# eloj/radix-sorting

Measured on AMD Instinct MI355X. Metric: Gkeys/s sorting 2^28 u32 (1 GPU) + HBM GB/s vs roofline; 1/2/4/8-GPU scaling, higher is better.
Workload: dtype u32

## Files before the change

radix_sorting_amd/csrc/rsx.hip:

```cpp
#include "../../include/rsx.h"
#include "rsx_kernels.hpp"
#include "rsx_scatter2.hpp"
#include "rsx_small.hpp"
#include "rsx_hybrid.hpp"
#include "rsx_leaf16.hpp"
#include "rsx_pass16.hpp"
#include "rsx_pass32.hpp"
#include "rsx_leafc.hpp"
#include "rsx_logroute.hpp"
#include "rsx_pass64.hpp"
#include "rsx_unique.hpp"
#include "rsx_group.hpp"
#include "rsx_topk.hpp"
#include "rsx_nth.hpp"
#include "rsx_lex.hpp"

#include <hip/hip_runtime.h>

#include <algorithm>
#include <cstdarg>
#include <cstdio>
#include <cstdlib>
#include <cstring>
#include <map>
// ... 653 lines not shown
}

template <typename KT> constexpr u64 seg_extra_rows() { return sizeof(KT) == 8 ? 512 : 256; }

template <typename KT> bool pass64a_narrow_wanted(const Ctx &c)
{
	if (sizeof(KT) != 8 || !narrow_slots_ok<KT>(c.slack_cap) || env().no_pass64a || env().no_unstable || !c.slack_mean)
		return false;
	u32 r = 0;
	while ((u64)(r + 1) * (r + 1) <= c.slack_mean)
		++r;
	return c.slack_mean + 6 * (r + 1) + 8 <= c.slack_cap - Pass2wCfg<u32>::BACK;
}

template <typename KT>
int launch_seg_pass(Ctx &c, const KT *aux, KT *src, size_t n, KdfArgs<KT> ka, int j, int blind = 0)
{
	typedef Sc2Cfg<KT, NoVal> C2;
	const u64 rows = (n + C2::TILE - 1) / C2::TILE + seg_extra_rows<KT>();
	const size_t st_bytes = 256 + rows * 256 * 4;
	char *base = (char *)c.seg.p + c.seg_status_off + (size_t)(blind == 1 ? 1 : j < 0 ? 0 : j) * st_bytes;
	SegArgs sa{};
	sa.ctl = (const SegCtl *)c.seg.p;
	sa.hist = (const u32 *)((char *)c.seg.p + c.seg_hist_off);
	sa.tiles = (const SegTile *)((char *)c.seg.p + c.seg_tiles_off);
	sa.slots = (u32)sizeof(KT) - 1;
	sa.slack_cap = blind == 1 ? c.slack1_cap : j == -2 ? c.slack_cap : 0u;
	sa.overflow = &((SegCtl *)c.seg.p)->overflow;
	KT *const second = blind == 1 ? src : blind == 2 ? const_cast<KT *>(aux) : nullptr;
	if (j == -2)
		src = (KT *)c.slack.p;
// ... 6 lines not shown
				const uintptr_t base_a = std::min(lo_a, hi_a);
				sa.out_off_lo = (u32)((lo_a - base_a) / sizeof(KT));
				sa.out_off_hi = (u32)((hi_a - base_a) / sizeof(KT));
				first = (KT *)base_a;
			} else {
				sa.kin_hi = (const void *)hi_a;
				first = second;
			}
		}
		if (blind == 1)
			src = first;
		else
			aux = first;
	}
	const bool dense = sizeof(KT) == 4 && blind == 2 && dense_slots<KT>(c);
	ProfScope prof(dense ? 3 : 1, (u64)n * (dense ? sizeof(KT) + 2 : 2 * sizeof(KT)), c.stream);
	const bool plain = ka.fmask == 0 && ka.sflip == 0 && ka.desc == 0;
	u32 flags = j == -2 ? (u32)SCATTER_SEG_SLACK : j < 0 ? (u32)SCATTER_SEG_LEAVES : 0u;
	if (blind)
		flags |= SCATTER_BLIND | (blind == 1 ? (u32)SCATTER_BLIND_TOP : 0u);
	if (blind && !env().no_unstable)
		flags |= SCATTER_UNSTABLE;
	const u32 pi = j < 0 ? 0u : (u32)j;
	const unsigned grid = blind == 1 ? (unsigned)(rows - seg_extra_rows<KT>()) : (unsigned)rows;
	const u32 shift0 = 0u;
#define RSX_LAUNCH_SEG(DIGV)                                                                                               \
	hipLaunchKernelGGL((rsx_scatter2_kernel<KT, NoVal, u32, C2, false, DIGV, false, KT, true>), dim3(grid),                 \
	                   dim3(C2::BLOCK), 0, c.stream, aux, src, (const NoVal *)nullptr, (NoVal *)nullptr, (u64)n, shift0,     \
	                   (const u64 *)c.ghist(), 1u, (u32 *)(base + 256), (u32 *)base, ka, flags, (u64 *)nullptr,             \
	                   (const Plan *)c.plan(), pi, 0u, (const u32 *)nullptr, sa)
	if constexpr (sizeof(KT) == 4) {
		if (dense && pass16a_wanted<KT>(c)) {
			const unsigned pgrid = 512;
			if (plain)
				hipLaunchKernelGGL((rsx_pass16a_kernel<KT, DIG_PLAIN>), dim3(pgrid), dim3(Pass16aCfg::BLOCK), 0, c.stream, (const KT *)aux,
				                   (const KT *)sa.kin_hi, sa.lo_slots, (unsigned short *)src, sa.tiles, sa.ctl, (const Plan *)c.plan(),
				                   (u32 *)(base + 256), sa.slack_cap, sa.overflow, ka);
			else
				hipLaunchKernelGGL((rsx_pass16a_kernel<KT, DIG_GENERIC>), dim3(pgrid), dim3(Pass16aCfg::BLOCK), 0, c.stream, (const KT *)aux,
				                   (const KT *)sa.kin_hi, sa.lo_slots, (unsigned short *)src, sa.tiles, sa.ctl, (const Plan *)c.plan(),
				                   (u32 *)(base + 256), sa.slack_cap, sa.overflow, ka);
			HIP_TRY(hipGetLastError());
			return RSX_OK;
		}
		if (dense && !env().no_pass16 && !env().no_unstable && !env().no_leaf16) {
			const u32 *btile = (const u32 *)((char *)c.seg.p + c.seg_btile_off);
#define RSX_LAUNCH_P16(DIGV, CFG)                                                                                          \
	hipLaunchKernelGGL((rsx_pass16_kernel<KT, DIGV, CFG>), dim3(grid), dim3(CFG::BLOCK), 0, c.stream, (const KT *)aux,      \
	                   (const KT *)sa.kin_hi, sa.lo_slots, (unsigned short *)src, sa.tiles, btile, sa.ctl,                  \
// ... 358 lines not shown
	u32 *btile = (u32 *)((char *)c.seg.p + c.seg_btile_off);
	u64 *off1 = (u64 *)c.gscan.p;
	if (!c.seg_ev && !c.small.external)
		HIP_TRY(hipEventCreateWithFlags(&c.seg_ev, hipEventDisableTiming));
	if (c.host_segctl)
		c.host_segctl->mode = SEG_MODE_NONE;
	c.slack1_cap = cap1;
	c.slack_cap = cap2;
	const bool atoms = pass16a_wanted<KT>(c);
	const bool atoms64 = pass64a_narrow_wanted<KT>(c);
	typedef Pass32aCfgT<sizeof(KT) == 8 ? 14 : 28> P32;
	const size_t min32 = env().pass32_min_mi ? (size_t)env().pass32_min_mi << 20 : sizeof(KT) == 8 ? (size_t)3 << 23 : (size_t)13 << 22;
	const bool atoms1 = (sizeof(KT) == 4 ? atoms : !env().no_unstable) && !env().no_pass32a && n >= min32 &&
	                    cap1 >= (u32)P32::TILE + 2 * PASS32_BACK;
	const bool rep4 = (c.hints & 1u) != 0 || (env().probe & 4u) != 0;
	c.narrow1 = sizeof(KT) == 8 && atoms1 && atoms64 && lo != 0 && !rep4 && !env().no_narrow1 && (((uintptr_t)aux) & 63) == 0 &&
	            (size_t)256 * cap1 * 4 <= n * sizeof(KT);
	static_assert(sizeof(SegCtl) <= 256, "the control block is not part of what is zeroed");
	RSX_TRY(blind_forget_device_backoff(c));
	hipLaunchKernelGGL((rsx_blind_precheck_kernel<KT>), dim3(1 + 512), dim3(1024), 0, c.stream, (const KT *)src, (u64)n, ka, ctl,
	                   c.plan(), c.dev_host_plan, (u32x4 *)((char *)c.seg.p + c.seg_status_off), (u64)(2 * st_bytes / 16),
	                   4u,
	                   (u32)(sizeof(KT) == 4 && dense_slots<KT>(c) && !env().no_leaf16 && !env().no_shift ? 1 : 0),
	                   (u32)(narrow_slots_ok<KT>(cap2) ? (c.narrow1 ? 2 : 1) : 0), 0u,
	                   (u32)(g_in_async ? 1 : 0), (u32)((env().probe & 4u) ? 1u : c.hints));
	{
		if (atoms1) {
			u32 off_lo = 0, off_hi = 0;
			KT *kbase = (KT *)c.slack1.p;
			if (lo) {
				const uintptr_t lo_a = (uintptr_t)aux, hi_a = (uintptr_t)c.slack1.p - (size_t)lo * cap1 * sizeof(KT);
				const uintptr_t base_a = std::min(lo_a, hi_a);
				off_lo = (u32)((lo_a - base_a) / sizeof(KT));
				off_hi = (u32)((hi_a - base_a) / sizeof(KT));
				kbase = (KT *)base_a;
			}
			u32 *cur1 = (u32 *)((char *)c.seg.p + c.seg_status_off + st_bytes + 256);
			u32 *ovf = &((SegCtl *)c.seg.p)->overflow;
			const bool plain = ka.fmask == 0 && ka.sflip == 0 && ka.desc == 0;
			ProfScope prof(1, (u64)n * 2 * sizeof(KT), c.stream);
			const bool prefetch = sizeof(KT) == 4 && env().pass32_prefetch > 0;
#define RSX_LAUNCH_P32R(DIGV, PF, REPV)                                                                                      \
			hipLaunchKernelGGL((rsx_pass32a_kernel<KT, DIGV, PF, P32, REPV>), dim3(256), dim3(P32::BLOCK), 0, c.stream,              \
			                   (const KT *)src, (u64)n, kbase, lo, off_lo, off_hi, cap1, (const SegCtl *)ctl, cur1, ovf, ka)
#define RSX_LAUNCH_P32(DIGV, PF)                                                                                             \
			do {                                                                                                                 \
				if (rep4 && !(PF))                                                                                               \
					RSX_LAUNCH_P32R(DIGV, false, 4);                                                                             \
				else                                                                                                             \
					RSX_LAUNCH_P32R(DIGV, PF, 1);                                                                                \
			} while (0)
			if constexpr (sizeof(KT) == 4) {
				if (plain && prefetch)
					RSX_LAUNCH_P32(DIG_PLAIN, true);
				else if (!plain && prefetch)
					RSX_LAUNCH_P32(DIG_GENERIC, true);
			}
			if (plain && !prefetch)
				RSX_LAUNCH_P32(DIG_PLAIN, false);
			else if (!prefetch)
				RSX_LAUNCH_P32(DIG_GENERIC, false);
#undef RSX_LAUNCH_P32
#undef RSX_LAUNCH_P32R
			if constexpr (sizeof(KT) == 8) {
				if (c.narrow1) {
					if (plain)
						hipLaunchKernelGGL((rsx_pass32a_kernel<KT, DIG_PLAIN, false, P32, 1, u32>), dim3(256), dim3(P32::BLOCK), 0, c.stream,
						                   (const KT *)src, (u64)n, (u32 *)aux, 256u, 0u, 0u, cap1, (const SegCtl *)ctl, cur1, ovf, ka);
					else
						hipLaunchKernelGGL((rsx_pass32a_kernel<KT, DIG_GENERIC, false, P32, 1, u32>), dim3(256), dim3(P32::BLOCK), 0, c.stream,
						                   (const KT *)src, (u64)n, (u32 *)aux, 256u, 0u, 0u, cap1, (const SegCtl *)ctl, cur1, ovf, ka);
				}
			}
			HIP_TRY(hipGetLastError());
		}
	}
	if (!atoms1)
		RSX_TRY(launch_seg_pass<KT>(c, src, lo ? aux : nullptr, n, ka, -2, 1));
	hipLaunchKernelGGL(rsx_seg_tiles_kernel, dim3(32), dim3(256), 0, c.stream, (const u64 *)c.ghist(), (u64)n, (const Plan *)c.plan(),
	                   atoms ? (u32)Pass16aCfg::TILE : (u32)C2::TILE, tiles, ctl, btile, off1, cap1,
	                   (const u32 *)((char *)c.seg.p + c.seg_status_off + st_bytes + 256), (u32)ntiles0, atoms1 ? PASS32_BACK : 0u,
	                   atoms64 ? (u32)Pass2wCfg<u32>::TILE : 0u, c.narrow1 ? (u32)Pass64aCfgLow::TILE : 0u);
	RSX_TRY(launch_seg_pass<KT>(c, lo ? aux : nullptr, nullptr, n, ka, -2, 2));
	hipLaunchKernelGGL((rsx_seg_slack_plan_kernel<u32>), dim3(256), dim3(256), 0, c.stream,
	                   (const u32 *)((char *)c.seg.p + c.seg_status_off + 256), (const u32 *)btile, (const u64 *)c.ghist(),
	                   (const Plan *)c.plan(), ctl, segtab, cap2, c.dev_host_segctl, (const u64 *)off1,
	                   (atoms ? 2u : atoms64 ? 3u : 1u) | ((env().probe & 1u) << 8));
	HIP_TRY(hipGetLastError());
	if (c.seg_ev)
		HIP_TRY(hipEventRecord(c.seg_ev, c.stream));
	u32 leaf_shape = LeafShapes<KT>::shape_for_slots(cap2);
	if (dense_slots<KT>(c))
		leaf_shape |= 0x100u;
	if (sizeof(KT) == 8 && cap2 <= 5120u)
		leaf_shape |= 0x200u;
	RSX_TRY(launch_leaves<KT>(c, src, aux, n, ka, HYB_TWO_LEVEL, leaf_shape, (const u64 *)off1));
	*enqueued = 1;
	return RSX_OK;
// ... 1961 lines not shown
```

radix_sorting_amd/csrc/rsx_env.hpp:

```cpp
#pragma once

#include <algorithm>
#include <atomic>
#include <climits>
#include <cstdint>
#include <cstdlib>
#include <mutex>

namespace {

std::atomic<uint32_t> g_env_epoch{0};
enum : unsigned { UNIQUE_MAX_BITS_COMPILED = 30, UNIQUE_MAX_BITS_DEFAULT = 24 };
enum : unsigned { GROUP_MAX_BITS_COMPILED = 30, GROUP_MAX_BITS_DEFAULT = 24 };
enum : unsigned { LEX_PACK_BYTES_DEFAULT = 4 };
struct Env {
	bool host_register = false;
	bool force_table_rank = false;
	bool verify = false;
	bool verify_whole = false;
	bool verify_inject = false;
	bool no_hot = false;
	bool elem_loads = false;
	bool no_small_tiles = false;
	bool no_hybrid = false;
	bool no_small_sort = false;
	bool no_fill_runs = false;
	bool no_speculation = false;
	bool compact_bits = false;
	bool no_narrow_keys = false;
// ... 8 lines not shown
	bool no_leaf16q = false;
	bool no_narrow_slots = false;
	bool no_aux_slots = false;
	bool no_narrow1 = false;
	bool no_dense_slots = false;
	bool force_dense_slots = false;
	bool no_unstable = false;
	bool no_shift = false;
	bool no_pass16 = false;
	unsigned pass16_wgs = 2;
	bool no_packed_keys = false;
	bool no_pass32a = false;
	unsigned pass32_min_mi = 0;
	int pass32_prefetch = -1;
	bool no_pass16a = false;
	unsigned pass16_dbg = 0;
	bool no_leafc = false;
	unsigned force_leafc = 0;
	bool no_leaf16 = false;
	unsigned leaf16_maxbin = 25;
	unsigned leaf_grid = 65536;
	unsigned two_level_min_log2 = 27;
	bool no_odd_stride = false;
	unsigned cap1_pad_kib = 0;
	unsigned probe = 0;
	bool no_pass64a = false;
	bool no_log = false;
	bool log_leaf_big = false;
	bool pairs_leaf_big = false;
	unsigned log_min_log2 = 0;
// ... 55 lines not shown
		no_narrow1 = is_one("RSX_NO_NARROW_LEVEL1");
		no_dense_slots = is_one("RSX_NO_DENSE_SLOTS");
		force_dense_slots = is_one("RSX_DENSE_SLOTS");
		no_leaf16 = is_one("RSX_NO_LEAF16");
		no_leafc = is_one("RSX_NO_LEAFC");
		no_leaf16w2k = is_one("RSX_NO_LEAF16W2K");
		number("RSX_PASS32_MIN_MI", &pass32_min_mi);
		if (is_set("RSX_PASS32_PREFETCH"))
			pass32_prefetch = is_one("RSX_PASS32_PREFETCH");
		number("RSX_FORCE_LEAFC", &force_leafc);
		no_pass16 = is_one("RSX_NO_PASS16");
		no_pass16a = is_one("RSX_NO_PASS16A");
		no_pass32a = is_one("RSX_NO_PASS32A");
		no_packed_keys = is_one("RSX_NO_PACKED_KEYS");
		one_else_two("RSX_PASS16_WGS", &pass16_wgs);
		number("RSX_PASS16_DBG", &pass16_dbg);
		no_shift = is_one("RSX_NO_SHIFT");
		no_unstable = is_one("RSX_NO_UNSTABLE");
		number("RSX_LEAF16_MAXBIN", &leaf16_maxbin, 0, 25);
		number("RSX_LEAF_GRID", &leaf_grid, 256, 65536);
		no_odd_stride = is_one("RSX_NO_ODD_STRIDE");
		number("RSX_CAP1_PAD_KIB", &cap1_pad_kib, 0, 65536);
		number("RSX_PROBE", &probe);
		no_pass64a = is_one("RSX_NO_PASS64A");
		no_log = is_one("RSX_NO_LOG");
		log_leaf_big = is_one("RSX_LOG_LEAF_BIG");
		pairs_leaf_big = is_one("RSX_PAIRS_LEAF_BIG");
		number("RSX_LOG_MIN_LOG2", &log_min_log2, 20, 29);
		topk_force = one_or_two("RSX_TOPK_FORCE");
		nth_force = one_or_two("RSX_NTH_FORCE");
// ... 16 lines not shown
```

radix_sorting_amd/csrc/rsx_pass16.hpp:

```cpp
#pragma once

#include "rsx_kernels.hpp"
#include "rsx_hybrid.hpp"

namespace rsx {

template <int WGS_ = 2> struct Pass16Cfg {
	static constexpr int WGS = WGS_;
	static constexpr int BLOCK = 1024, KPT = 32, TILE = BLOCK * KPT;
	static constexpr int NGROUP = TILE / 8;
};

template <int WGS> struct Pass16Smem {
	__attribute__((aligned(16))) unsigned short stage[32768 + (WGS == 1 ? 8192 : 0)];
	u32 cell[256];
	u32 delta[256];
	unsigned short rend[256];
	unsigned char group_digit[4096];
	u32 wsum[4];
};

template <typename KT, int DIG, typename C = Pass16Cfg<2>>
__global__ __launch_bounds__(C::BLOCK, C::WGS * 4) void rsx_pass16_kernel(const KT *__restrict__ kin, const KT *__restrict__ kin_hi,
                                                                         u32 lo_slots, unsigned short *__restrict__ kout,
// ... 164 lines not shown
	static constexpr u32 BACK = 128;
	static constexpr int STAGE = TILE + 256 * 14;
};

struct Pass16aSmem {
	__attribute__((aligned(16))) unsigned short stage[Pass16aCfg::STAGE];
	__attribute__((aligned(16))) unsigned short carry[256][32];
	u32 cell[2][256];
	u32 delta[256];
	u32 info[256];
	unsigned short rbeg[256], bbeg[256], bend[256];
	unsigned char group_digit[Pass16aCfg::STAGE / 8];
	u32 wsum[4];
};

template <typename KT, int DIG, bool PREFETCH = false>
__global__ __launch_bounds__(Pass16aCfg::BLOCK, 8) void rsx_pass16a_kernel(const KT *__restrict__ kin, const KT *__restrict__ kin_hi,
                                                                          u32 lo_slots, unsigned short *__restrict__ kout,
                                                                          const SegTile *__restrict__ tiles,
                                                                          const SegCtl *__restrict__ ctl,
                                                                          const Plan *__restrict__ plan, u32 *__restrict__ cursors,
                                                                          u32 slack_cap, u32 *__restrict__ overflow, KdfArgs<KT> ka)
{
	static_assert(sizeof(KT) == 4, "4-byte keys, two-byte values");
	typedef Pass16aCfg C;
	constexpr int BLOCK = C::BLOCK, KPT = C::KPT, TILE = C::TILE;
	if (ctl->blind != BLIND_GO || plan->hyb != HYB_TWO_LEVEL)
		return;
	const u32 ntiles = ctl->ntiles;
	const u32 per = (ntiles + gridDim.x - 1) / gridDim.x;
	const u32 t0 = blockIdx.x * per, t1 = t0 + per < ntiles ? t0 + per : ntiles;
	if (t0 >= t1)
		return;
	const u32 shift = ctl->shift2;
	const u32 gran = ctl->leaf16 ? C::ATOM : 1u;
	__shared__ Pass16aSmem sm;
	const u32 tid0 = threadIdx.x;
	auto sidx = [](u32 pos) { return stage_swz<true>(pos * 2u); };
	auto staged = [&](u32 pos) -> unsigned short & { return *(unsigned short *)((char *)sm.stage + sidx(pos)); };
// ... 22 lines not shown
		}
		__syncthreads();
		{
			const u32 n = sm.info[cd], dest = sm.delta[cd];
#pragma unroll 2
			for (u32 e = 0; e < 8; ++e) {
				const u32 k = part * 8u + e;
				if (k < n)
					kout[dest + k] = sm.carry[cd][k];
			}
		}
		__syncthreads();
	};
	__syncthreads();
	KT keep[KPT];
	auto request = [&](const u32 t, const u32 tid) {
		const SegTile st = tiles[t];
		const KT *p = ((kin_hi && st.bucket >= lo_slots) ? kin_hi : kin) + st.beg;
		if (st.cnt == (u32)TILE && (((uintptr_t)p) & 15) == 0) {
			typedef KT vec_t __attribute__((ext_vector_type(4)));
			const vec_t *vp = (const vec_t *)p + tid;
#pragma unroll
			for (int i = 0; i < KPT / 4; ++i) {
				const vec_t v = __builtin_nontemporal_load(&vp[i * BLOCK]);
#pragma unroll
				for (int e = 0; e < 4; ++e)
					keep[4 * i + e] = v[e];
			}
		} else {
#pragma unroll
			for (int r = 0; r < KPT; ++r) {
				const u32 o = tid + r * BLOCK;
// ... 17 lines not shown
			bucket = st.bucket;
		}
		const u32 cnt = st.cnt;
		const bool full = cnt == (u32)TILE;
		if constexpr (!PREFETCH)
			request(t, tid);
		if constexpr (DIG != 1) {
#pragma unroll
			for (int r = 0; r < KPT; ++r)
				keep[r] = kdf_apply(keep[r], ka);
		}
		auto count = [&](auto full_c) {
			constexpr bool FULL = decltype(full_c)::value;
#pragma unroll
			for (int r = 0; r < KPT; ++r) {
				if (FULL || tid + r * BLOCK < cnt)
					atomicAdd(&cell[(u32)(keep[r] >> shift) & 0xFFu], 1u);
			}
		};
		if (full)
			count(std::true_type{});
		else
			count(std::false_type{});
		__syncthreads();

		u32 base = 0;
		{
			u32 rlen = 0, rstart = 0;
			if (tid < 256) {
				const u32 c = cell[tid];
				u32 h, body = 0, tail = 0, atom = 0;
				const bool enough = cc + c >= gran;
// ... 41 lines not shown
		}
		__syncthreads();

		if (tid < 256) {
			const u32 slot = bucket * 256u + tid;
			const u32 atom = (sm.info[tid] >> 18) & 1u, bb = sm.bbeg[tid], m = atom * gran + (sm.bend[tid] - bb);
			u32 dest = slot * slack_cap + base + atom * gran;
			if (m && base + m > slack_cap - C::BACK) {
				atomicOr(overflow, 1u);
				dest = 65536u * slack_cap + C::ATOM;
			}
			sm.delta[tid] = dest - bb;
		}
		u32 shift_b = shift;
		asm volatile("" : "+s"(shift_b));
		auto stage_keys = [&](auto full_c) {
			constexpr bool FULL = decltype(full_c)::value;
#pragma unroll
			for (int r0 = 0; r0 < KPT; r0 += 8) {
				u32 pos[8];
#pragma unroll
				for (int r = 0; r < 8; ++r) {
					pos[r] = 0;
					if (FULL || tid + (r0 + r) * BLOCK < cnt)
						pos[r] = __hip_atomic_fetch_add(&cell[(u32)(keep[r0 + r] >> shift_b) & 0xFFu], 1u, __ATOMIC_RELAXED,
						                                __HIP_MEMORY_SCOPE_WORKGROUP);
				}
#pragma unroll
				for (int r = 0; r < 8; ++r) {
					if (FULL || tid + (r0 + r) * BLOCK < cnt)
						staged(pos[r]) = (unsigned short)keep[r0 + r];
				}
			}
		};
		if (full)
			stage_keys(std::true_type{});
		else
			stage_keys(std::false_type{});
		__syncthreads();

		if constexpr (PREFETCH) {
			if (t + 1 < t1)
				request(t + 1, tid);
		}
		{
			const u32 inf = sm.info[cd];
// ... 61 lines not shown
```

radix_sorting_amd/csrc/rsx_pass32.hpp:

```cpp
#pragma once

#include "rsx_kernels.hpp"
#include "rsx_hybrid.hpp"
#include "rsx_scatter2.hpp"

namespace rsx {

template <int KPT_ = 28, bool RANK1_ = true> struct Pass32aCfgT {
	static constexpr int BLOCK = 1024, KPT = KPT_, TILE = BLOCK * KPT;
	static constexpr bool RANK1 = RANK1_;
	static constexpr int WPE = KPT_ <= 12 ? 8 : 4;
	static constexpr int SB = KPT_ % 7 == 0 ? 7 : 6;
	static constexpr u32 ATOM = 16;
	static constexpr u32 BACK = 8192;
	static constexpr int STAGE = TILE + 256 * 6;
};
typedef Pass32aCfgT<28> Pass32aCfg;
constexpr u32 PASS32_BACK = Pass32aCfg::BACK;

template <typename KT, typename C, int REP = 1> struct Pass32aSmem {
	__attribute__((aligned(16))) KT stage[C::STAGE];
	__attribute__((aligned(16))) KT carry[256][64 / sizeof(KT)];
	__attribute__((aligned(16))) u32 cell[2][256 * REP];
	u32 delta[256];
	u32 info[256];
	unsigned short rbeg[256], bbeg[256], bend[256];
	unsigned char group_digit[C::STAGE / (16 / sizeof(KT))];
	u32 wsum[4];
};

template <typename KT, int DIG, bool PREFETCH = true, typename C = Pass32aCfg, int REP_ = 1, typename OT = KT>
__global__ __launch_bounds__(C::BLOCK, C::WPE) void rsx_pass32a_kernel(const KT *__restrict__ kin, u64 n, OT *__restrict__ kout,
                                                                          u32 lo_slots, u32 off_lo, u32 off_hi, u32 cap,
                                                                          const SegCtl *__restrict__ ctl,
                                                                          u32 *__restrict__ cursors, u32 *__restrict__ overflow,
                                                                          KdfArgs<KT> ka)
{
	static_assert(sizeof(KT) == 4 || sizeof(KT) == 8, "4- or 8-byte keys");
	constexpr int BLOCK = C::BLOCK, KPT = C::KPT, TILE = C::TILE, SB = C::SB;
	constexpr u32 VIN = 16 / sizeof(KT);
	constexpr u32 VEC = 16 / sizeof(OT);
	constexpr u32 ATOM = 64 / sizeof(OT);
	constexpr bool NARROW = sizeof(OT) != sizeof(KT);
	static_assert(!NARROW || (sizeof(KT) == 8 && sizeof(OT) == 4), "8-byte keys into four-byte slots, or the element images");
	static_assert(KPT % (int)VIN == 0, "whole vectors per lane");
	static_assert(sizeof(OT) == 4 || C::STAGE * sizeof(OT) + 256 * 64 <= 150 * 1024, "8-byte slots: 14 Ki-key tiles (Pass32aCfgT<14>)");
	if (ctl->blind != BLIND_GO)
		return;
	if constexpr (sizeof(KT) == 8) {
		if ((ctl->narrow == 2u) != NARROW)
			return;
	}
	const u32 ntiles = (u32)((n + TILE - 1) / TILE);
	const u32 per = (ntiles + gridDim.x - 1) / gridDim.x;
	const u32 t0 = blockIdx.x * per, t1 = t0 + per < ntiles ? t0 + per : ntiles;
	if (t0 >= t1)
		return;
	const u32 shift = ctl->shift1;
	const KT cmask = sizeof(KT) == 8 ? (KT)(((u64)ctl->cmask_hi << 32) | ctl->cmask_lo) : (KT)ctl->cmask_lo;
	const KT key0 = sizeof(KT) == 8 ? (KT)(((u64)ctl->key0_hi << 32) | ctl->key0_lo) : (KT)ctl->key0_lo;
	__shared__ Pass32aSmem<OT, C, REP_> sm;
	const u32 tid0 = threadIdx.x;
	auto sidx = [](u32 pos) { return stage_swz<true>(pos * (u32)sizeof(OT)); };
	auto staged = [&](u32 pos) -> OT & { return *(OT *)((char *)sm.stage + sidx(pos)); };
	auto slot_base = [&](u32 d) { return (d < lo_slots ? off_lo : off_hi) + d * cap; };
	u32 cc = 0;
	constexpr u32 REP = REP_;
	static_assert(REP == 1 || REP == 4, "one counter per digit, or one per lane class");
	if (tid0 < 256 * REP)
		sm.cell[0][tid0] = 0;
	__syncthreads();
	auto bucket_of = [&](KT k, u32 sh) -> u32 { return (u32)(k >> sh) & 0xFFu; };
	KT keep[KPT];
	auto request = [&](const u32 t, const u32 tid) {
		const u64 beg = (u64)t * TILE;
		const u32 cnt = n - beg < (u64)TILE ? (u32)(n - beg) : (u32)TILE;
		const KT *p = kin + beg;
		if (cnt == (u32)TILE && (((uintptr_t)p) & 15) == 0) {
			typedef KT vec_t __attribute__((ext_vector_type(VIN)));
// ... 68 lines not shown
				u32 h, body = 0, tail = 0, atom = 0;
				const bool enough = cc + c >= ATOM;
				if (enough) {
					h = cc ? ATOM - cc : 0u;
					atom = cc ? 1u : 0u;
					body = (c - h) & ~(ATOM - 1u);
					tail = (c - h) & (ATOM - 1u);
				} else {
					h = c;
				}
				const u32 m = atom * ATOM + body;
				if (m)
					base = __hip_atomic_fetch_add(cursors + tid, m, __ATOMIC_RELAXED, __HIP_MEMORY_SCOPE_AGENT);
				const u32 o = (VEC - (h & (VEC - 1u))) & (VEC - 1u);
				rlen = (o + c + VEC - 1u) & ~(VEC - 1u);
				sm.info[tid] = cc | (h << 5) | (tail << 10) | (atom << 15) | ((enough ? 1u : 0u) << 16) | (o << 17);
				sm.bend[tid] = (unsigned short)body;
				cc = enough ? tail : cc + c;
				u32 x = rlen;
#pragma unroll
				for (int off = 1; off < 64; off <<= 1) {
					const u32 y = __shfl_up(x, off);
					if (lane >= (u32)off)
						x += y;
				}
				if (lane == 63)
					sm.wsum[wid] = x;
				rstart = x - rlen;
			}
			__syncthreads();
			if (tid < 256) {
				for (u32 k = 0; k < wid; ++k)
					rstart += sm.wsum[k];
				const u32 inf = sm.info[tid];
				const u32 rb = rstart + (inf >> 17), bb = rb + ((inf >> 5) & 31u), be = bb + sm.bend[tid];
				u32 rq = rb;
#pragma unroll
				for (u32 q = 0; q < REP; ++q) {
					cell[tid * REP + q] = rq;
					rq += crep[q];
					sm.cell[((t - t0) & 1u) ^ 1u][tid * REP + q] = 0;
				}
				sm.rbeg[tid] = (unsigned short)rb;
				sm.bbeg[tid] = (unsigned short)bb;
				sm.bend[tid] = (unsigned short)be;
				for (u32 g = bb / VEC; g < (be + VEC - 1u) / VEC; ++g)
					sm.group_digit[g] = (unsigned char)tid;
			}
		}
		__syncthreads();

		if (tid < 256) {
			const u32 atom = (sm.info[tid] >> 15) & 1u, bb = sm.bbeg[tid], m = atom * ATOM + (sm.bend[tid] - bb);
			u32 dest = slot_base(tid) + base + atom * ATOM;
			if (m && base + m > cap - C::BACK) {
				atomicOr(overflow, 1u);
				dest = slot_base(tid) + ATOM;
			}
			sm.delta[tid] = dest - bb;
		}
		u32 shift_b = shift;
		asm volatile("" : "+s"(shift_b));
		auto stage_keys = [&](auto full_c) {
			constexpr bool FULL = decltype(full_c)::value;
#pragma unroll
			for (int r0 = 0; r0 < KPT; r0 += SB) {
				u32 pos[SB];
#pragma unroll
				for (int r = 0; r < SB; ++r) {
					pos[r] = 0;
					if (FULL || tid + (r0 + r) * BLOCK < cnt) {
						const KT k = DIG == 1 ? keep[r0 + r] : kdf_apply(keep[r0 + r], ka);
						const u32 b = bucket_of(k, shift_b) * REP + (lane & (REP - 1u));
						if constexpr (C::RANK1)
							pos[r] = cell[b] + ((rk[(r0 + r) >> 1] >> (16 * ((r0 + r) & 1))) & 0xFFFFu);
						else
							pos[r] = __hip_atomic_fetch_add(&cell[b], 1u, __ATOMIC_RELAXED, __HIP_MEMORY_SCOPE_WORKGROUP);
					}
				}
#pragma unroll
				for (int r = 0; r < SB; ++r) {
					if (FULL || tid + (r0 + r) * BLOCK < cnt) {
						if constexpr (NARROW)
							staged(pos[r]) = (OT)(DIG == 1 ? keep[r0 + r] : kdf_apply(keep[r0 + r], ka));
						else
							staged(pos[r]) = keep[r0 + r];
					}
				}
			}
		};
		if (full)
			stage_keys(std::true_type{});
		else
			stage_keys(std::false_type{});
		__syncthreads();
		if constexpr (PREFETCH) {
			if (t + 1 < t1)
				request(t + 1, tid);
		}

		{
			const u32 inf = sm.info[cd];
			const u32 ccd = inf & 31u, atomd = (inf >> 15) & 1u;
			if (atomd) {
				const u32 rb = sm.rbeg[cd];
				typedef OT kvec_t __attribute__((ext_vector_type(VEC)));
				typedef kvec_t avec_t __attribute__((aligned(16)));
				kvec_t w;
#pragma unroll
				for (u32 e = 0; e < VEC; ++e) {
					const u32 k = part * VEC + e;
					w[e] = k < ccd ? sm.carry[cd][k] : staged(rb + (k - ccd));
				}
				*(avec_t *)(kout + (u32)(sm.delta[cd] + sm.bbeg[cd] - ATOM + part * VEC)) = w;
			}
		}
		{
			const u32 total = (u32)__builtin_amdgcn_readfirstlane((int)sm.wsum[0]) + sm.wsum[1] + sm.wsum[2] + sm.wsum[3];
#pragma unroll 1
			for (u32 i0 = VEC * tid; i0 < total; i0 += VEC * BLOCK) {
				const u32 d = sm.group_digit[i0 / VEC];
				if (i0 >= sm.bbeg[d] && i0 < sm.bend[d]) {
					typedef OT kvec_t __attribute__((ext_vector_type(VEC)));
					typedef kvec_t avec_t __attribute__((aligned(16)));
					*(avec_t *)(kout + (u32)(sm.delta[d] + i0)) = *(const kvec_t *)((const char *)sm.stage + sidx(i0));
				}
			}
		}
		{
			const u32 inf = sm.info[cd];
			const u32 ccd = inf & 31u, hd = (inf >> 5) & 31u, taild = (inf >> 10) & 31u, enoughd = (inf >> 16) & 1u;
			const u32 from = enoughd ? sm.bend[cd] : sm.rbeg[cd], to = enoughd ? 0u : ccd, nk = enoughd ? taild : hd;
#pragma unroll
			for (u32 e = 0; e < VEC; ++e) {
				const u32 k = part * VEC + e;
				if (k < nk)
					sm.carry[cd][to + k] = staged(from + k);
			}
		}
	}
	{
		const u32 tid = tid0, cd = tid >> 2, part = tid & 3u;
		__syncthreads();
		if (tid < 256) {
			u32 inf = 0, dest = 0;
			if (cc) {
				const u32 pos = __hip_atomic_fetch_add(cursors + 256u + tid, cc, __ATOMIC_RELAXED, __HIP_MEMORY_SCOPE_AGENT);
				if (pos + cc > C::BACK)
					atomicOr(overflow, 1u);
				else {
					inf = cc;
					dest = slot_base(tid) + (cap - C::BACK) + pos;
				}
			}
			sm.info[tid] = inf;
			sm.delta[tid] = dest;
		}
		__syncthreads();
		const u32 nk = sm.info[cd], dest = sm.delta[cd];
#pragma unroll
		for (u32 e = 0; e < VEC; ++e) {
			const u32 k = part * VEC + e;
			if (k < nk)
				kout[dest + k] = sm.carry[cd][k];
		}
	}
}

}
```

Before: 216.2.

## Pack first-pass intermediate keys into 24-bit grouped slots to cut HBM traffic

After the top-byte pass, each remaining key needs only its low 24 bits. This change stores them in 64-key groups laid out as 128 bytes of 16-bit halves followed by 64 bytes of 8-bit mids. The pass32a scatter writes this packed format and pass16a reads it back, so the intermediate write and read each move 3 bytes per key instead of 4. The cost is more complex LDS staging, larger atom and backstop sizes, and extra carry handling, and the packed path runs only under alignment and size conditions.

```diff
diff --git a/radix_sorting_amd/csrc/rsx.hip b/radix_sorting_amd/csrc/rsx.hip
--- a/radix_sorting_amd/csrc/rsx.hip
+++ b/radix_sorting_amd/csrc/rsx.hip
@@ -691,7 +691,7 @@
 }
 
 template <typename KT>
-int launch_seg_pass(Ctx &c, const KT *aux, KT *src, size_t n, KdfArgs<KT> ka, int j, int blind = 0)
+int launch_seg_pass(Ctx &c, const KT *aux, KT *src, size_t n, KdfArgs<KT> ka, int j, int blind = 0, bool pack24 = false)
 {
 	typedef Sc2Cfg<KT, NoVal> C2;
 	const u64 rows = (n + C2::TILE - 1) / C2::TILE + seg_extra_rows<KT>();
@@ -728,7 +728,7 @@
 			aux = first;
 	}
 	const bool dense = sizeof(KT) == 4 && blind == 2 && dense_slots<KT>(c);
-	ProfScope prof(dense ? 3 : 1, (u64)n * (dense ? sizeof(KT) + 2 : 2 * sizeof(KT)), c.stream);
+	ProfScope prof(dense ? 3 : 1, (u64)n * (dense ? (pack24 ? 3 : sizeof(KT)) + 2 : 2 * sizeof(KT)), c.stream);
 	const bool plain = ka.fmask == 0 && ka.sflip == 0 && ka.desc == 0;
 	u32 flags = j == -2 ? (u32)SCATTER_SEG_SLACK : j < 0 ? (u32)SCATTER_SEG_LEAVES : 0u;
 	if (blind)
@@ -746,7 +746,11 @@
 	if constexpr (sizeof(KT) == 4) {
 		if (dense && pass16a_wanted<KT>(c)) {
 			const unsigned pgrid = 512;
-			if (plain)
+			if (pack24)
+				hipLaunchKernelGGL((rsx_pass16a_kernel<KT, DIG_PLAIN, false, true>), dim3(pgrid), dim3(Pass16aCfg::BLOCK), 0, c.stream, (const KT *)aux,
+				                   (const KT *)sa.kin_hi, sa.lo_slots, (unsigned short *)src, sa.tiles, sa.ctl, (const Plan *)c.plan(),
+				                   (u32 *)(base + 256), sa.slack_cap, sa.overflow, KdfArgs<KT>{0, 0, 0}, c.slack1_cap);
+			else if (plain)
 				hipLaunchKernelGGL((rsx_pass16a_kernel<KT, DIG_PLAIN>), dim3(pgrid), dim3(Pass16aCfg::BLOCK), 0, c.stream, (const KT *)aux,
 				                   (const KT *)sa.kin_hi, sa.lo_slots, (unsigned short *)src, sa.tiles, sa.ctl, (const Plan *)c.plan(),
 				                   (u32 *)(base + 256), sa.slack_cap, sa.overflow, ka);
@@ -1135,6 +1139,11 @@
 	const bool atoms1 = (sizeof(KT) == 4 ? atoms : !env().no_unstable) && !env().no_pass32a && n >= min32 &&
 	                    cap1 >= (u32)P32::TILE + 2 * PASS32_BACK;
 	const bool rep4 = (c.hints & 1u) != 0 || (env().probe & 4u) != 0;
+	typedef Pass32aCfg24<24> P24;
+	bool pack24 = false;
+	if constexpr (sizeof(KT) == 4)
+		pack24 = atoms1 && atoms && !rep4 && !env().no_pack24 && env().pass32_prefetch <= 0 && (((uintptr_t)aux | (uintptr_t)c.slack1.p) & 63) == 0 &&
+		         n <= ((size_t)1 << 29) && n >= ((size_t)env().pack24_min_mi << 20) && cap1 % 64u == 0 && cap1 >= (u32)P24::TILE + 2 * P24::BACK;
 	c.narrow1 = sizeof(KT) == 8 && atoms1 && atoms64 && lo != 0 && !rep4 && !env().no_narrow1 && (((uintptr_t)aux) & 63) == 0 &&
 	            (size_t)256 * cap1 * 4 <= n * sizeof(KT);
 	static_assert(sizeof(SegCtl) <= 256, "the control block is not part of what is zeroed");
@@ -1159,7 +1168,7 @@
 			u32 *cur1 = (u32 *)((char *)c.seg.p + c.seg_status_off + st_bytes + 256);
 			u32 *ovf = &((SegCtl *)c.seg.p)->overflow;
 			const bool plain = ka.fmask == 0 && ka.sflip == 0 && ka.desc == 0;
-			ProfScope prof(1, (u64)n * 2 * sizeof(KT), c.stream);
+			ProfScope prof(1, (u64)n * (pack24 ? 7 : 2 * sizeof(KT)), c.stream);
 			const bool prefetch = sizeof(KT) == 4 && env().pass32_prefetch > 0;
 #define RSX_LAUNCH_P32R(DIGV, PF, REPV)                                                                                      \
 			hipLaunchKernelGGL((rsx_pass32a_kernel<KT, DIGV, PF, P32, REPV>), dim3(256), dim3(P32::BLOCK), 0, c.stream,              \
@@ -1172,12 +1181,20 @@
 					RSX_LAUNCH_P32R(DIGV, PF, 1);                                                                                \
 			} while (0)
 			if constexpr (sizeof(KT) == 4) {
-				if (plain && prefetch)
+				if (pack24 && plain)
+					hipLaunchKernelGGL((rsx_pass32a_kernel<KT, DIG_PLAIN, false, P24, 1, Pack24>), dim3(256), dim3(P24::BLOCK), 0, c.stream,
+					                   (const KT *)src, (u64)n, (Pack24 *)kbase, lo, off_lo, off_hi, cap1, (const SegCtl *)ctl, cur1, ovf, ka);
+				else if (pack24)
+					hipLaunchKernelGGL((rsx_pass32a_kernel<KT, DIG_GENERIC, false, P24, 1, Pack24>), dim3(256), dim3(P24::BLOCK), 0, c.stream,
+					                   (const KT *)src, (u64)n, (Pack24 *)kbase, lo, off_lo, off_hi, cap1, (const SegCtl *)ctl, cur1, ovf, ka);
+				else if (plain && prefetch)
 					RSX_LAUNCH_P32(DIG_PLAIN, true);
 				else if (!plain && prefetch)
 					RSX_LAUNCH_P32(DIG_GENERIC, true);
 			}
-			if (plain && !prefetch)
+			if (pack24)
+				;
+			else if (plain && !prefetch)
 				RSX_LAUNCH_P32(DIG_PLAIN, false);
 			else if (!prefetch)
 				RSX_LAUNCH_P32(DIG_GENERIC, false);
@@ -1200,9 +1217,9 @@
 		RSX_TRY(launch_seg_pass<KT>(c, src, lo ? aux : nullptr, n, ka, -2, 1));
 	hipLaunchKernelGGL(rsx_seg_tiles_kernel, dim3(32), dim3(256), 0, c.stream, (const u64 *)c.ghist(), (u64)n, (const Plan *)c.plan(),
 	                   atoms ? (u32)Pass16aCfg::TILE : (u32)C2::TILE, tiles, ctl, btile, off1, cap1,
-	                   (const u32 *)((char *)c.seg.p + c.seg_status_off + st_bytes + 256), (u32)ntiles0, atoms1 ? PASS32_BACK : 0u,
+	                   (const u32 *)((char *)c.seg.p + c.seg_status_off + st_bytes + 256), (u32)ntiles0, atoms1 ? (pack24 ? P24::BACK : PASS32_BACK) : 0u,
 	                   atoms64 ? (u32)Pass2wCfg<u32>::TILE : 0u, c.narrow1 ? (u32)Pass64aCfgLow::TILE : 0u);
-	RSX_TRY(launch_seg_pass<KT>(c, lo ? aux : nullptr, nullptr, n, ka, -2, 2));
+	RSX_TRY(launch_seg_pass<KT>(c, lo ? aux : nullptr, nullptr, n, ka, -2, 2, pack24));
 	hipLaunchKernelGGL((rsx_seg_slack_plan_kernel<u32>), dim3(256), dim3(256), 0, c.stream,
 	                   (const u32 *)((char *)c.seg.p + c.seg_status_off + 256), (const u32 *)btile, (const u64 *)c.ghist(),
 	                   (const Plan *)c.plan(), ctl, segtab, cap2, c.dev_host_segctl, (const u64 *)off1,
diff --git a/radix_sorting_amd/csrc/rsx_env.hpp b/radix_sorting_amd/csrc/rsx_env.hpp
--- a/radix_sorting_amd/csrc/rsx_env.hpp
+++ b/radix_sorting_amd/csrc/rsx_env.hpp
@@ -13,6 +13,7 @@
 enum : unsigned { UNIQUE_MAX_BITS_COMPILED = 30, UNIQUE_MAX_BITS_DEFAULT = 24 };
 enum : unsigned { GROUP_MAX_BITS_COMPILED = 30, GROUP_MAX_BITS_DEFAULT = 24 };
 enum : unsigned { LEX_PACK_BYTES_DEFAULT = 4 };
+enum : unsigned { PACK24_MIN_MI_DEFAULT = 1u << 20 };
 struct Env {
 	bool host_register = false;
 	bool force_table_rank = false;
@@ -51,6 +52,8 @@
 	unsigned pass32_min_mi = 0;
 	int pass32_prefetch = -1;
 	bool no_pass16a = false;
+	bool no_pack24 = false;
+	unsigned pack24_min_mi = PACK24_MIN_MI_DEFAULT;
 	unsigned pass16_dbg = 0;
 	bool no_leafc = false;
 	unsigned force_leafc = 0;
@@ -136,6 +139,8 @@
 		no_pass32a = is_one("RSX_NO_PASS32A");
 		no_packed_keys = is_one("RSX_NO_PACKED_KEYS");
 		one_else_two("RSX_PASS16_WGS", &pass16_wgs);
+		no_pack24 = is_one("RSX_NO_PACK24");
+		number("RSX_PACK24_MIN_MI", &pack24_min_mi, 1, 1 << 20);
 		number("RSX_PASS16_DBG", &pass16_dbg);
 		no_shift = is_one("RSX_NO_SHIFT");
 		no_unstable = is_one("RSX_NO_UNSTABLE");
diff --git a/radix_sorting_amd/csrc/rsx_pack24.hpp b/radix_sorting_amd/csrc/rsx_pack24.hpp
--- /dev/null
+++ b/radix_sorting_amd/csrc/rsx_pack24.hpp
@@ -0,0 +1,52 @@
+#pragma once
+
+#include <cstdint>
+
+#if defined(__HIPCC__) || defined(__CUDACC__)
+#define RSX_PACK24_HD __host__ __device__ __forceinline__
+#else
+#define RSX_PACK24_HD inline
+#endif
+
+namespace rsx {
+namespace pack24 {
+
+constexpr uint32_t GROUP = 64;
+constexpr uint32_t GROUP_BYTES = 192;
+constexpr uint32_t MID_OFF = 128;
+constexpr uint32_t QUARTER = 16;
+
+RSX_PACK24_HD uint64_t group_byte(uint64_t i) { return (i >> 6) * GROUP_BYTES; }
+RSX_PACK24_HD uint64_t half_byte(uint64_t i) { return group_byte(i) + 2u * (i & 63u); }
+RSX_PACK24_HD uint64_t mid_byte(uint64_t i) { return group_byte(i) + MID_OFF + (i & 63u); }
+RSX_PACK24_HD uint64_t slot_bytes(uint64_t nkeys) { return (nkeys + GROUP - 1) / GROUP * GROUP_BYTES; }
+
+RSX_PACK24_HD void store_key(unsigned char *slot, uint64_t i, uint32_t key)
+{
+	*(unsigned short *)(slot + half_byte(i)) = (unsigned short)key;
+	slot[mid_byte(i)] = (unsigned char)(key >> 16);
+}
+RSX_PACK24_HD uint32_t load_key(const unsigned char *slot, uint64_t i)
+{
+	return (uint32_t)*(const unsigned short *)(slot + half_byte(i)) | ((uint32_t)slot[mid_byte(i)] << 16);
+}
+
+RSX_PACK24_HD void pack_quarter(unsigned char *slot, uint64_t i0, const uint32_t *keys, uint32_t nk = QUARTER)
+{
+	unsigned short *h = (unsigned short *)(slot + half_byte(i0));
+	unsigned char *m = slot + mid_byte(i0);
+	for (uint32_t e = 0; e < nk; ++e) {
+		h[e] = (unsigned short)keys[e];
+		m[e] = (unsigned char)(keys[e] >> 16);
+	}
+}
+RSX_PACK24_HD void unpack_quarter(const unsigned char *slot, uint64_t i0, uint32_t *keys, uint32_t nk = QUARTER)
+{
+	const unsigned short *h = (const unsigned short *)(slot + half_byte(i0));
+	const unsigned char *m = slot + mid_byte(i0);
+	for (uint32_t e = 0; e < nk; ++e)
+		keys[e] = (uint32_t)h[e] | ((uint32_t)m[e] << 16);
+}
+
+}
+}
diff --git a/radix_sorting_amd/csrc/rsx_pass16.hpp b/radix_sorting_amd/csrc/rsx_pass16.hpp
--- a/radix_sorting_amd/csrc/rsx_pass16.hpp
+++ b/radix_sorting_amd/csrc/rsx_pass16.hpp
@@ -2,6 +2,7 @@
 
 #include "rsx_kernels.hpp"
 #include "rsx_hybrid.hpp"
+#include "rsx_pack24.hpp"
 
 namespace rsx {
 
@@ -202,15 +203,17 @@
 	u32 wsum[4];
 };
 
-template <typename KT, int DIG, bool PREFETCH = false>
+template <typename KT, int DIG, bool PREFETCH = false, bool PACK24 = false>
 __global__ __launch_bounds__(Pass16aCfg::BLOCK, 8) void rsx_pass16a_kernel(const KT *__restrict__ kin, const KT *__restrict__ kin_hi,
                                                                           u32 lo_slots, unsigned short *__restrict__ kout,
                                                                           const SegTile *__restrict__ tiles,
                                                                           const SegCtl *__restrict__ ctl,
                                                                           const Plan *__restrict__ plan, u32 *__restrict__ cursors,
-                                                                          u32 slack_cap, u32 *__restrict__ overflow, KdfArgs<KT> ka)
+                                                                          u32 slack_cap, u32 *__restrict__ overflow, KdfArgs<KT> ka,
+                                                                          u32 cap1 = 0)
 {
 	static_assert(sizeof(KT) == 4, "4-byte keys, two-byte values");
+	static_assert(!PACK24 || (DIG == 1 && Pass16aCfg::KPT % 8 == 0), "packed slots hold derived keys; eight keys per lane and round");
 	typedef Pass16aCfg C;
 	constexpr int BLOCK = C::BLOCK, KPT = C::KPT, TILE = C::TILE;
 	if (ctl->blind != BLIND_GO || plan->hyb != HYB_TWO_LEVEL)
@@ -263,8 +266,41 @@
 	};
 	__syncthreads();
 	KT keep[KPT];
+	auto key_index = [](const u32 tid, const int r) -> u32 {
+		return PACK24 ? 8u * (tid + (u32)(r >> 3) * BLOCK) + (u32)(r & 7) : tid + (u32)r * BLOCK;
+	};
+	auto key_of = [&](const int r) -> KT {
+		if constexpr (PACK24) {
+			const int j = r >> 3, e = r & 7;
+			return ((keep[4 * j + (e >> 1)] >> (16 * (e & 1))) & 0xFFFFu) | (((keep[KPT / 2 + 2 * j + (e >> 2)] >> (8 * (e & 3))) & 0xFFu) << 16);
+		} else
+			return keep[r];
+	};
 	auto request = [&](const u32 t, const u32 tid) {
 		const SegTile st = tiles[t];
+		if constexpr (PACK24) {
+			const unsigned char *slot = (const unsigned char *)((kin_hi && st.bucket >= lo_slots) ? kin_hi : kin) + (u64)st.bucket * cap1 * 4u;
+			const u32 in_slot = st.beg - st.bucket * cap1;
+			typedef u32 vec4_t __attribute__((ext_vector_type(4)));
+			typedef u32 vec2_t __attribute__((ext_vector_type(2)));
+#pragma unroll
+			for (int j = 0; j < KPT / 8; ++j) {
+				const u32 o = 8u * (tid + (u32)j * BLOCK);
+				vec4_t h = {0, 0, 0, 0};
+				vec2_t m = {0, 0};
+				if (o < st.cnt) {
+					const u64 i = (u64)in_slot + o;
+					h = __builtin_nontemporal_load((const vec4_t *)(slot + pack24::half_byte(i)));
+					m = __builtin_nontemporal_load((const vec2_t *)(slot + pack24::mid_byte(i)));
+				}
+#pragma unroll
+				for (int e = 0; e < 4; ++e)
+					keep[4 * j + e] = h[e];
+				keep[KPT / 2 + 2 * j] = m[0];
+				keep[KPT / 2 + 2 * j + 1] = m[1];
+			}
+			return;
+		}
 		const KT *p = ((kin_hi && st.bucket >= lo_slots) ? kin_hi : kin) + st.beg;
 		if (st.cnt == (u32)TILE && (((uintptr_t)p) & 15) == 0) {
 			typedef KT vec_t __attribute__((ext_vector_type(4)));
@@ -312,8 +348,8 @@
 			constexpr bool FULL = decltype(full_c)::value;
 #pragma unroll
 			for (int r = 0; r < KPT; ++r) {
-				if (FULL || tid + r * BLOCK < cnt)
-					atomicAdd(&cell[(u32)(keep[r] >> shift) & 0xFFu], 1u);
+				if (FULL || key_index(tid, r) < cnt)
+					atomicAdd(&cell[(u32)(key_of(r) >> shift) & 0xFFu], 1u);
 			}
 		};
 		if (full)
@@ -385,6 +421,11 @@
 		}
 		u32 shift_b = shift;
 		asm volatile("" : "+s"(shift_b));
+		if constexpr (PACK24) {
+#pragma unroll
+			for (int r = 0; r < KPT * 3 / 4; ++r)
+				asm volatile("" : "+v"(keep[r]));
+		}
 		auto stage_keys = [&](auto full_c) {
 			constexpr bool FULL = decltype(full_c)::value;
 #pragma unroll
@@ -393,14 +434,14 @@
 #pragma unroll
 				for (int r = 0; r < 8; ++r) {
 					pos[r] = 0;
-					if (FULL || tid + (r0 + r) * BLOCK < cnt)
-						pos[r] = __hip_atomic_fetch_add(&cell[(u32)(keep[r0 + r] >> shift_b) & 0xFFu], 1u, __ATOMIC_RELAXED,
+					if (FULL || key_index(tid, r0 + r) < cnt)
+						pos[r] = __hip_atomic_fetch_add(&cell[(u32)(key_of(r0 + r) >> shift_b) & 0xFFu], 1u, __ATOMIC_RELAXED,
 						                                __HIP_MEMORY_SCOPE_WORKGROUP);
 				}
 #pragma unroll
 				for (int r = 0; r < 8; ++r) {
-					if (FULL || tid + (r0 + r) * BLOCK < cnt)
-						staged(pos[r]) = (unsigned short)keep[r0 + r];
+					if (FULL || key_index(tid, r0 + r) < cnt)
+						staged(pos[r]) = (unsigned short)key_of(r0 + r);
 				}
 			}
 		};
diff --git a/radix_sorting_amd/csrc/rsx_pass32.hpp b/radix_sorting_amd/csrc/rsx_pass32.hpp
--- a/radix_sorting_amd/csrc/rsx_pass32.hpp
+++ b/radix_sorting_amd/csrc/rsx_pass32.hpp
@@ -3,6 +3,9 @@
 #include "rsx_kernels.hpp"
 #include "rsx_hybrid.hpp"
 #include "rsx_scatter2.hpp"
+#include "rsx_pack24.hpp"
+
+#include <type_traits>
 
 namespace rsx {
 
@@ -10,13 +13,22 @@
 	static constexpr int BLOCK = 1024, KPT = KPT_, TILE = BLOCK * KPT;
 	static constexpr bool RANK1 = RANK1_;
 	static constexpr int WPE = KPT_ <= 12 ? 8 : 4;
-	static constexpr int SB = KPT_ % 7 == 0 ? 7 : 6;
+	static constexpr int SB = KPT_ % 7 == 0 ? 7 : KPT_ % 6 == 0 ? 6 : 5;
 	static constexpr u32 ATOM = 16;
 	static constexpr u32 BACK = 8192;
 	static constexpr int STAGE = TILE + 256 * 6;
 };
 typedef Pass32aCfgT<28> Pass32aCfg;
 constexpr u32 PASS32_BACK = Pass32aCfg::BACK;
+
+struct Pack24 {
+	unsigned char b;
+};
+template <int KPT_ = 24> struct Pass32aCfg24 : Pass32aCfgT<KPT_, true> {
+	static constexpr u32 ATOM = 64;
+	static constexpr u32 BACK = 16384;
+	static constexpr int STAGE = Pass32aCfgT<KPT_, true>::TILE + 256 * 30;
+};
 
 template <typename KT, typename C, int REP = 1> struct Pass32aSmem {
 	__attribute__((aligned(16))) KT stage[C::STAGE];
@@ -28,6 +40,29 @@
 	unsigned char group_digit[C::STAGE / (16 / sizeof(KT))];
 	u32 wsum[4];
 };
+template <typename C, int REP> struct Pass32aSmem<Pack24, C, REP> {
+	__attribute__((aligned(16))) unsigned short stage_lo[C::STAGE];
+	__attribute__((aligned(16))) unsigned char stage_mid[C::STAGE];
+	__attribute__((aligned(16))) unsigned short carry_lo[256][64];
+	__attribute__((aligned(16))) unsigned char carry_mid[256][64];
+	u32 cell[2][256 * REP];
+	u32 delta[256];
+	u32 info[256];
+	unsigned short rbeg[256], bbeg[256], bend[256];
+	unsigned char group_digit[C::STAGE / 16];
+	u32 wsum[4];
+};
+static_assert(sizeof(Pass32aSmem<Pack24, Pass32aCfg24<24>, 1>) <= 150 * 1024 && sizeof(Pass32aSmem<Pack24, Pass32aCfg24<20>, 1>) <= 150 * 1024,
+              "one workgroup per CU");
+
+template <typename SM> __device__ __forceinline__ unsigned short &pack24_lo(SM &sm, u32 pos)
+{
+	return *(unsigned short *)((char *)sm.stage_lo + stage_swz<true>(pos * 2u));
+}
+template <typename SM> __device__ __forceinline__ unsigned char &pack24_mid(SM &sm, u32 pos)
+{
+	return *((unsigned char *)sm.stage_mid + stage_swz<true>(pos));
+}
 
 template <typename KT, int DIG, bool PREFETCH = true, typename C = Pass32aCfg, int REP_ = 1, typename OT = KT>
 __global__ __launch_bounds__(C::BLOCK, C::WPE) void rsx_pass32a_kernel(const KT *__restrict__ kin, u64 n, OT *__restrict__ kout,
@@ -39,12 +74,16 @@
 	static_assert(sizeof(KT) == 4 || sizeof(KT) == 8, "4- or 8-byte keys");
 	constexpr int BLOCK = C::BLOCK, KPT = C::KPT, TILE = C::TILE, SB = C::SB;
 	constexpr u32 VIN = 16 / sizeof(KT);
+	constexpr bool PACK = std::is_same<OT, Pack24>::value;
 	constexpr u32 VEC = 16 / sizeof(OT);
 	constexpr u32 ATOM = 64 / sizeof(OT);
+	constexpr u32 FW = PACK ? 6 : 5;
+	constexpr u32 FM = (1u << FW) - 1u;
+	static_assert(!PACK || (sizeof(KT) == 4 && C::ATOM == ATOM && VEC == 16 && REP_ == 1), "4-byte keys into groups of 64");
 	constexpr bool NARROW = sizeof(OT) != sizeof(KT);
-	static_assert(!NARROW || (sizeof(KT) == 8 && sizeof(OT) == 4), "8-byte keys into four-byte slots, or the element images");
+	static_assert(PACK || !NARROW || (sizeof(KT) == 8 && sizeof(OT) == 4), "8-byte keys into four-byte slots, or the element images");
 	static_assert(KPT % (int)VIN == 0, "whole vectors per lane");
-	static_assert(sizeof(OT) == 4 || C::STAGE * sizeof(OT) + 256 * 64 <= 150 * 1024, "8-byte slots: 14 Ki-key tiles (Pass32aCfgT<14>)");
+	static_assert(PACK || sizeof(OT) == 4 || C::STAGE * sizeof(OT) + 256 * 64 <= 150 * 1024, "8-byte slots: 14 Ki-key tiles (Pass32aCfgT<14>)");
 	if (ctl->blind != BLIND_GO)
 		return;
 	if constexpr (sizeof(KT) == 8) {
@@ -62,7 +101,12 @@
 	__shared__ Pass32aSmem<OT, C, REP_> sm;
 	const u32 tid0 = threadIdx.x;
 	auto sidx = [](u32 pos) { return stage_swz<true>(pos * (u32)sizeof(OT)); };
-	auto staged = [&](u32 pos) -> OT & { return *(OT *)((char *)sm.stage + sidx(pos)); };
+	auto staged = [&](u32 pos) -> OT & {
+		if constexpr (PACK)
+			return *(OT *)&pack24_mid(sm, pos);
+		else
+			return *(OT *)((char *)sm.stage + sidx(pos));
+	};
 	auto slot_base = [&](u32 d) { return (d < lo_slots ? off_lo : off_hi) + d * cap; };
 	u32 cc = 0;
 	constexpr u32 REP = REP_;
@@ -161,7 +205,7 @@
 					base = __hip_atomic_fetch_add(cursors + tid, m, __ATOMIC_RELAXED, __HIP_MEMORY_SCOPE_AGENT);
 				const u32 o = (VEC - (h & (VEC - 1u))) & (VEC - 1u);
 				rlen = (o + c + VEC - 1u) & ~(VEC - 1u);
-				sm.info[tid] = cc | (h << 5) | (tail << 10) | (atom << 15) | ((enough ? 1u : 0u) << 16) | (o << 17);
+				sm.info[tid] = cc | (h << FW) | (tail << 2 * FW) | (atom << 3 * FW) | ((enough ? 1u : 0u) << (3 * FW + 1)) | (o << (3 * FW + 2));
 				sm.bend[tid] = (unsigned short)body;
 				cc = enough ? tail : cc + c;
 				u32 x = rlen;
@@ -180,7 +224,7 @@
 				for (u32 k = 0; k < wid; ++k)
 					rstart += sm.wsum[k];
 				const u32 inf = sm.info[tid];
-				const u32 rb = rstart + (inf >> 17), bb = rb + ((inf >> 5) & 31u), be = bb + sm.bend[tid];
+				const u32 rb = rstart + (inf >> (3 * FW + 2)), bb = rb + ((inf >> FW) & FM), be = bb + sm.bend[tid];
 				u32 rq = rb;
 #pragma unroll
 				for (u32 q = 0; q < REP; ++q) {
@@ -198,11 +242,12 @@
 		__syncthreads();
 
 		if (tid < 256) {
-			const u32 atom = (sm.info[tid] >> 15) & 1u, bb = sm.bbeg[tid], m = atom * ATOM + (sm.bend[tid] - bb);
-			u32 dest = slot_base(tid) + base + atom * ATOM;
+			const u32 atom = (sm.info[tid] >> 3 * FW) & 1u, bb = sm.bbeg[tid], m = atom * ATOM + (sm.bend[tid] - bb);
+			const u32 sbase = PACK ? 0u : slot_base(tid);
+			u32 dest = sbase + base + atom * ATOM;
 			if (m && base + m > cap - C::BACK) {
 				atomicOr(overflow, 1u);
-				dest = slot_base(tid) + ATOM;
+				dest = sbase + ATOM;
 			}
 			sm.delta[tid] = dest - bb;
 		}
@@ -228,7 +273,11 @@
 #pragma unroll
 				for (int r = 0; r < SB; ++r) {
 					if (FULL || tid + (r0 + r) * BLOCK < cnt) {
-						if constexpr (NARROW)
+						if constexpr (PACK) {
+							const u32 k = (u32)(DIG == 1 ? keep[r0 + r] : kdf_apply(keep[r0 + r], ka));
+							pack24_lo(sm, pos[r]) = (unsigned short)k;
+							pack24_mid(sm, pos[r]) = (unsigned char)(k >> 16);
+						} else if constexpr (NARROW)
 							staged(pos[r]) = (OT)(DIG == 1 ? keep[r0 + r] : kdf_apply(keep[r0 + r], ka));
 						else
 							staged(pos[r]) = keep[r0 + r];
@@ -248,8 +297,44 @@
 
 		{
 			const u32 inf = sm.info[cd];
-			const u32 ccd = inf & 31u, atomd = (inf >> 15) & 1u;
-			if (atomd) {
+			const u32 ccd = inf & FM, atomd = (inf >> 3 * FW) & 1u;
+			if constexpr (PACK) {
+				if (atomd) {
+					const u32 bb = sm.bbeg[cd];
+					auto halves = [&](const u32 k0) -> u32x4 {
+						const u32x4 a = *(const u32x4 *)&sm.carry_lo[cd][k0];
+						const u32 sp = k0 + 8u > ccd ? bb - 64u + k0 : bb - 16u;
+						const u32x4 b = *(const u32x4 *)((const char *)sm.stage_lo + stage_swz<true>(sp * 2u));
+						u32x4 r;
+#pragma unroll
+						for (u32 e = 0; e < 4; ++e) {
+							const u32 kk = k0 + 2u * e, m = kk + 1u < ccd ? 0xFFFFFFFFu : kk < ccd ? 0xFFFFu : 0u;
+							r[e] = (a[e] & m) | (b[e] & ~m);
+						}
+						return r;
+					};
+					auto mids = [&](const u32 k0) -> u32x4 {
+						const u32x4 a = *(const u32x4 *)&sm.carry_mid[cd][k0];
+						const u32 sp = k0 + 16u > ccd ? bb - 64u + k0 : bb - 16u;
+						const u32x4 b = *(const u32x4 *)((const char *)sm.stage_mid + stage_swz<true>(sp));
+						u32x4 r;
+#pragma unroll
+						for (u32 e = 0; e < 4; ++e) {
+							const u32 kk = k0 + 4u * e, nb = ccd > kk ? (ccd - kk < 4u ? ccd - kk : 4u) : 0u;
+							const u32 m = nb >= 4u ? 0xFFFFFFFFu : (1u << (8u * nb)) - 1u;
+							r[e] = (a[e] & m) | (b[e] & ~m);
+						}
+						return r;
+					};
+					const u32x4 h0 = halves(part * 8u), h1 = halves(32u + part * 8u), mm = mids(part * 16u);
+					typedef u32x4 avec_t __attribute__((aligned(16)));
+					const u32 idx = sm.delta[cd] + sm.bbeg[cd] - ATOM;
+					unsigned char *gp = (unsigned char *)kout + (u64)slot_base(cd) * 4u + pack24::group_byte(idx);
+					*(avec_t *)(gp + 16u * part) = h0;
+					*(avec_t *)(gp + 64u + 16u * part) = h1;
+					*(avec_t *)(gp + pack24::MID_OFF + 16u * part) = mm;
+				}
+			} else if (atomd) {
 				const u32 rb = sm.rbeg[cd];
 				typedef OT kvec_t __attribute__((ext_vector_type(VEC)));
 				typedef kvec_t avec_t __attribute__((aligned(16)));
@@ -267,7 +352,20 @@
 #pragma unroll 1
 			for (u32 i0 = VEC * tid; i0 < total; i0 += VEC * BLOCK) {
 				const u32 d = sm.group_digit[i0 / VEC];
-				if (i0 >= sm.bbeg[d] && i0 < sm.bend[d]) {
+				if constexpr (PACK) {
+					const u32 bb = sm.bbeg[d];
+					if (i0 >= bb && i0 < sm.bend[d]) {
+						const u32 rel = i0 - bb, q = (rel >> 4) & 3u, sg = i0 - 16u * q;
+						typedef u32x4 avec_t __attribute__((aligned(16)));
+						const u32x4 h0 = *(const u32x4 *)((const char *)sm.stage_lo + stage_swz<true>((sg + 8u * q) * 2u));
+						const u32x4 h1 = *(const u32x4 *)((const char *)sm.stage_lo + stage_swz<true>((sg + 32u + 8u * q) * 2u));
+						const u32x4 mm = *(const u32x4 *)((const char *)sm.stage_mid + stage_swz<true>(sg + 16u * q));
+						unsigned char *gp = (unsigned char *)kout + (u64)slot_base(d) * 4u + pack24::group_byte(sm.delta[d] + sg);
+						*(avec_t *)(gp + 16u * q) = h0;
+						*(avec_t *)(gp + 64u + 16u * q) = h1;
+						*(avec_t *)(gp + pack24::MID_OFF + 16u * q) = mm;
+					}
+				} else if (i0 >= sm.bbeg[d] && i0 < sm.bend[d]) {
 					typedef OT kvec_t __attribute__((ext_vector_type(VEC)));
 					typedef kvec_t avec_t __attribute__((aligned(16)));
 					*(avec_t *)(kout + (u32)(sm.delta[d] + i0)) = *(const kvec_t *)((const char *)sm.stage + sidx(i0));
@@ -276,12 +374,25 @@
 		}
 		{
 			const u32 inf = sm.info[cd];
-			const u32 ccd = inf & 31u, hd = (inf >> 5) & 31u, taild = (inf >> 10) & 31u, enoughd = (inf >> 16) & 1u;
+			const u32 ccd = inf & FM, hd = (inf >> FW) & FM, taild = (inf >> 2 * FW) & FM, enoughd = (inf >> (3 * FW + 1)) & 1u;
 			const u32 from = enoughd ? sm.bend[cd] : sm.rbeg[cd], to = enoughd ? 0u : ccd, nk = enoughd ? taild : hd;
+			if constexpr (PACK) {
+				if (enoughd && part * 16u < taild) {
+					const u32 f = from + part * 16u;
+					*(u32x4 *)&sm.carry_lo[cd][part * 16u] = *(const u32x4 *)((const char *)sm.stage_lo + stage_swz<true>(f * 2u));
+					*(u32x4 *)&sm.carry_lo[cd][part * 16u + 8u] = *(const u32x4 *)((const char *)sm.stage_lo + stage_swz<true>((f + 8u) * 2u));
+					*(u32x4 *)&sm.carry_mid[cd][part * 16u] = *(const u32x4 *)((const char *)sm.stage_mid + stage_swz<true>(f));
+				}
+			}
 #pragma unroll
 			for (u32 e = 0; e < VEC; ++e) {
 				const u32 k = part * VEC + e;
-				if (k < nk)
+				if constexpr (PACK) {
+					if (!enoughd && k < nk) {
+						sm.carry_lo[cd][to + k] = pack24_lo(sm, from + k);
+						sm.carry_mid[cd][to + k] = pack24_mid(sm, from + k);
+					}
+				} else if (k < nk)
 					sm.carry[cd][to + k] = staged(from + k);
 			}
 		}
@@ -297,7 +408,7 @@
 					atomicOr(overflow, 1u);
 				else {
 					inf = cc;
-					dest = slot_base(tid) + (cap - C::BACK) + pos;
+					dest = (PACK ? 0u : slot_base(tid)) + (cap - C::BACK) + pos;
 				}
 			}
 			sm.info[tid] = inf;
@@ -308,7 +419,10 @@
 #pragma unroll
 		for (u32 e = 0; e < VEC; ++e) {
 			const u32 k = part * VEC + e;
-			if (k < nk)
+			if constexpr (PACK) {
+				if (k < nk)
+					pack24::store_key((unsigned char *)kout + (u64)slot_base(cd) * 4u, dest + k, (u32)sm.carry_lo[cd][k] | ((u32)sm.carry_mid[cd][k] << 16));
+			} else if (k < nk)
 				kout[dest + k] = sm.carry[cd][k];
 		}
 	}
```

New measurement: 216.3, median of 2. About the same (+0.0%).
